# dojo-sim/ContactImplicitMPC.jl

Hardware: AMD Instinct MI355X
Metric: MPC steps/s (quadruped, H=40, fp64) (higher is better)
Workload: dtype f64

## Files before the change

contactimplicitmpc/jl_amd/csrc/cimpc_host.cpp:

```cpp
#include <hip/hip_runtime.h>

#include <algorithm>
#include <chrono>
#include <cmath>
#include <cstdio>
#include <cstdlib>
#include <cstring>
#include <string>
#include <vector>

#include "cimpc_internal.h"
#include "lin_table.h"
#include "lin_table_build.h"
#include "model_table.h"
#include "newton_state.h"
#include "gains.h"
#include "handle_state.h"
#include "plant_linearize.h"
#include "schedule_plan.h"

using namespace cimpc;

namespace {

// ... 26 lines not shown
    int kkt_tw_spins = 0;
    int banded_form = 0;

    static int env_int(const char* name, int dflt) { const char* v = getenv(name); return v ? atoi(v) : dflt; }
    void read_environment() {
        sched.async_mode = env_int("CIMPC_ASYNC", sched.async_mode);
        sched.async_tail = env_int("CIMPC_ASYNC_TAIL", sched.async_tail);
        sched.spec_first = env_int("CIMPC_SPEC_FIRST", sched.spec_first);
        sched.iter_cap = std::max(1, env_int("CIMPC_ITER_CAP", sched.iter_cap));
        async_debug = getenv("CIMPC_ASYNC_DEBUG") != nullptr;
        if (const char* v = getenv("CIMPC_ASYNC_WATCHDOG_S")) watchdog_s = atof(v);
        debug_rounds = getenv("CIMPC_DEBUG_ROUNDS") != nullptr;
        sched.tail_div = env_int("CIMPC_TAIL_DIV", sched.tail_div);
        sched.async_full_max = env_int("CIMPC_ASYNC_FULL_MAX", sched.async_full_max);
        sched.drain_pct = env_int("CIMPC_DRAIN_PCT", sched.drain_pct);
        sched.drain_min = std::max(1, env_int("CIMPC_DRAIN_MIN", sched.drain_min));
        kkt.kkt_pipe = env_int("CIMPC_KKT_PIPE", kkt.kkt_pipe);
        kkt.kkt_twisted = env_int("CIMPC_KKT_TWISTED", kkt.kkt_twisted);
        kkt_tw_nb = env_int("CIMPC_KKT_TW_NB", kkt_tw_nb);
        kkt.lazy_dz = env_int("CIMPC_LAZY_DZ", 1) != 0;
        kkt.kkt_duo = env_int("CIMPC_KKT_DUO", kkt.kkt_duo);
        kkt.kkt_duo_hint = env_int("CIMPC_KKT_DUO_HINT", kkt.kkt_duo_hint);
        kkt.async_kkt_tw = env_int("CIMPC_ASYNC_KKT_TW", kkt.async_kkt_tw);
        generic_static = env_int("CIMPC_GENERIC_STATIC", generic_static ? 1 : 0) != 0;
        sched.sweep_wgs = env_int("CIMPC_SWEEP_WGS", sched.sweep_wgs);
        sched.waves32 = env_int("CIMPC_WAVES32", sched.waves32);
        banded_form = env_int("CIMPC_BANDED_FORM", banded_form);
    }
};

struct cimpc_ctx {
    cimpc_dims dm{};
    Knobs kn{};
    cimpc_ip_opts ip{};
    cimpc_newton_opts nt{};
    int device = 0;
    hipStream_t stream = nullptr;
    bool own_stream = false;
    std::string err;
    KernelInfo ki{};
    int nz = 0, nth = 0, nths = 0, nd = 0, nr = 0, nx = 0, ny = 0, N = 0;
// ... 1056 lines not shown
    if (from_reset) h->prof_kkt_systems += h->last_stats.newton_iters;
    return CIMPC_OK;
}

int launch_round(cimpc_ctx* h, SolveRun& run, long long r, bool blind) {
    const RoundStreams& sb = run.sb; const RoundCounts& last = run.last;
    const int par = (int)(r & 1);
    h->S.kkt_tw_epoch += 1;
    const bool tw_off = note_tw_fallbacks(h) != run.tw_fail0;
    NewtonDev Sk = launch_view(h, par);
    Sk.A.n_done = run.hybrid ? h->a_ctrl + async_ctl(h->Q.K).n_done : nullptr;
    Sk.round_stamp = (int)(r + 1);
    const bool kkt = (r > 0) && (blind || last.kkt > 0);
    const int n_kkt = blind ? h->dm.B : last.kkt;
    const int* n_kkt_dev = blind ? round_counter(Sk.counters_next, RC_KKT) : nullptr;
    if (kkt) {
        const bool ov = h->kp.kkt_overlap;
        const KktSite site{.kind = ov ? KktSite::Overlapped : KktSite::Round, .n_kkt = n_kkt, .blind = blind,
                           .sweep_problems = (long long)last.new_slots * h->dm.H, .tw_off = tw_off, .B = h->dm.B};
        hipStream_t kst = ov ? sb.st_kkt : sb.st;
        if (!ov) Sk.kkt_same_round = 1;
        prof_begin(h, PC_KKT, kst);
        int rk = run_kkt_stage(h, Sk, kkt_newton_args(Sk), site, Sk.kkt_list + (size_t)(par ^ 1) * h->dm.B,
                               ov ? last.kkt : n_kkt, ov ? nullptr : n_kkt_dev, kst);
        prof_end(h, kst);
        if (rk != CIMPC_OK) return fail(h, rk, "kkt launch failed");
        if (ov && hipEventRecord(sb.ev_join, sb.st_kkt) != hipSuccess) return fail(h, CIMPC_ERR_HIP, "join record failed");
    }
    const RoundPlan rp = plan_round(h->kn.sched, h->sched, h->ip.max_iter, kkt, blind, last.sweep, last.slots);
    const long long hint = blind ? -1 : (long long)last.slots * h->dm.H + last.parked;
    if (h->kn.debug_rounds && !blind) print_queued_problems(h, run, r, par, hint);
    int rr = run_sweep(h, par, round_counter(Sk.counters, RC_PARKED), nullptr, sb.st, rp.cap, round_counter(Sk.counters, RC_DRAINED), true, hint);
    if (rr != CIMPC_OK) return rr;
    prof_begin(h, PC_RESID, sb.st);
    if (rp.split_join) {
        rr = launch_resid_decide(Sk, sb.st, rp.n_slots, 1);
        if (rr != CIMPC_OK) return fail(h, rr, "residual launch failed");
    }
    if (kkt && h->kp.kkt_overlap && hipStreamWaitEvent(sb.st, sb.ev_join, 0) != hipSuccess) return fail(h, CIMPC_ERR_HIP, "join failed");
    rr = launch_resid_decide(Sk, sb.st, rp.n_slots, rp.split_join ? 2 : 0);
    prof_end(h, sb.st);
    if (rr != CIMPC_OK) return fail(h, rr, "residual launch failed");
    return CIMPC_OK;
}

}

int cimpc_newton_solve_dev(cimpc_handle h, const double* q0_dev, const double* q1_dev, int warm_start) {
    int rc = check_ready(h, true);
    if (rc != CIMPC_OK) return rc;
    if (!q0_dev || !q1_dev) return fail(h, CIMPC_ERR_INVALID, "null argument");
    HIP_TRY(h, hipSetDevice(h->device));
    if (int sy = sync_dz_stores(h, DZ_NEWTON); sy != CIMPC_OK) return sy;
    h->st.solve_started();
// ... 25 lines not shown
    while (true) {
        if (completed >= round_limit) {
            (void)hipStreamSynchronize(sb.st); (void)hipStreamSynchronize(sb.st_kkt);
            return fail(h, CIMPC_ERR_STATE, "newton_solve: round limit reached with unfinished rollouts");
        }
        while (launched <= completed + (ahead ? 1 : 0)) {
            rc = launch_round(h, run, launched, launched > completed);
            if (rc != CIMPC_OK) return rc;
            ++launched;
        }
        {
            volatile int* hm = ring_slot((volatile int*)h->h_ring, completed);
            const int want = (int)(completed + 1);
            long long spins = 0;
            while (hm[RING_STAMP] != want) {
                if ((++spins & 0xFFFFF) == 0 && hipStreamQuery(sb.st) != hipErrorNotReady && hm[RING_STAMP] != want)
                    return fail(h, CIMPC_ERR_HIP, "round finished without publishing its counters");
            }
        }
        const RoundCounts& last = run.last = read_round_counts(h->h_ring, completed);
        if (h->kn.debug_rounds) fprintf(stderr, "[cimpc round %lld] t %.3f ms: next sweep %d rollouts (%d evaluation slots), next kkt %d, parked %d, finished %d\n", completed,
                                        1e3 * elapsed_s(run), last.sweep, last.slots, last.kkt, last.parked, last.finished);
        h->prof_kkt_systems += last.kkt;
        ++completed;
        if ((last.sweep == 0 && last.kkt == 0) || over_budget(h, run)) break;
        if (run.hybrid && hand_over(h->sched, B - last.finished)) {
            HIP_TRY(h, hipStreamSynchronize(sb.st));
            HIP_TRY(h, hipStreamSynchronize(sb.st_kkt));
            return run_async(h, run, false, completed);
        }
    }
// ... 377 lines not shown
```

contactimplicitmpc/jl_amd/csrc/newton_impl.h:

```cpp
#pragma once
#include "lane_group.h"
#include "newton_state.h"

namespace cimpc {

struct BlockSync { static __device__ __forceinline__ void sync() { __syncthreads(); } };
struct WaveSync {
    static __device__ __forceinline__ void sync() {
        __builtin_amdgcn_fence(__ATOMIC_SEQ_CST, "workgroup");
        __builtin_amdgcn_wave_barrier();
    }
};

__device__ __forceinline__ void theta_update(const NewtonDev& S, const TrajDev& T, int b, int i,
                                             int tid, int nthreads) {
    const cimpc_dims& m = S.dm;
    double* th = T.th + ((size_t)b * m.H + i) * S.nth;
    const double* q = T.q + ((size_t)b * (m.H + 2) + i) * m.nq;
    const double* u = T.u + ((size_t)b * m.H + i) * m.nu;
    const double* w = T.w + ((size_t)b * m.H + i) * m.nw;
    for (int k = tid; k < 2 * m.nq; k += nthreads) th[k] = q[k];
    for (int k = tid; k < m.nu; k += nthreads) th[2 * m.nq + k] = u[k];
    for (int k = tid; k < m.nw; k += nthreads) th[2 * m.nq + m.nu + k] = w[k];
}
// ... 13 lines not shown

__device__ __forceinline__ void enqueue_eval(const NewtonDev& S, size_t sb, int b, int par, int tid, int nt, int list_pos = -1) {
    const int H = S.dm.H, K = S.WQ.K;
    for (int k = tid; k < H; k += nt) {
        const int t = S.WQ.window[(size_t)b * (H + 2) + k];
        const int pos = atomicAdd(qcount(S.WQ, par, t), 1);
        S.WQ.items[((size_t)par * K + t) * S.WQ.cap + pos] = (int)(sb * H + k);
    }
    if (tid == 0) {
        S.WQ.done_count[sb] = 0;
        S.need_sweep[sb] = 1;
        list_slot(S, sb, par, list_pos);
    }
}

__device__ __forceinline__ void enqueue_evals(const NewtonDev& S, size_t sb, int n, int b, int par, int tid, int nt, int mark = 1) {
    const int H = S.dm.H, K = S.WQ.K;
    for (int k = tid; k < H; k += nt) {
        const int t = S.WQ.window[(size_t)b * (H + 2) + k];
        const int pos = atomicAdd(qcount(S.WQ, par, t), n);
        int* it = S.WQ.items + ((size_t)par * K + t) * S.WQ.cap + pos;
        for (int c = 0; c < n; ++c) it[c] = (int)((sb + c) * H + k);
    }
    if (tid == 0) {
        int pos = 0;
        if (S.slot_list != nullptr) pos = atomicAdd(round_counter(S.counters, RC_SLOTS), n);
        atomicAdd(round_counter(S.counters, RC_NEW_SLOTS), n);
        if (pos + n > S.dm.B * CS) __builtin_trap();
        for (int c = 0; c < n; ++c) {
            S.WQ.done_count[sb + c] = 0;
            S.need_sweep[sb + c] = mark;
// ... 157 lines not shown
}

template <class Sync>
__device__ __forceinline__ void start_line_search(const NewtonDev& S, int b, int mode, int lane, int nt) {
    const size_t sb0 = (size_t)b * CS;
    int n = 1;
    {
        const int prev = S.ls_iter[b];
        if (S.newton_l[b] == 0) n = S.spec_first;
        else if (prev >= S.spec_all) n = 7;
        else if (prev >= S.spec_mid) n = 3;
        n = (n >= 7) ? 7 : (n >= 3) ? 3 : 1;
    }
    Sync::sync();
    apply_steps<Sync>(S, sb0, 0, n, b, lane, nt);
    if (lane == 0) { S.alpha[b] = 1.0; S.ls_iter[b] = 0; S.stage[b] = (n == 7) ? STAGE_LS7 : (n == 3) ? STAGE_LS3 : STAGE_LS0; }
    if (mode == 2) {
        enqueue_eval_async<Sync>(S, sb0, 0, n, b, lane, nt);
    } else {
        const int par = (S.kkt_same_round == 1) ? S.WQ.par : (S.WQ.par ^ 1);
        enqueue_evals(S, sb0, n, b, par, lane, nt, S.kkt_same_round == 0 ? 2 : 1);
        if (lane == 0) {
            for (int c = n; c < CS; ++c) S.need_sweep[sb0 + c] = 0;
            if (S.kkt_same_round == 0) atomicAdd(round_counter(S.counters, RC_SWEEP), 1);
        }
    }
}


__device__ __forceinline__ const double* dz_eff(const NewtonDev& S, int b, int it, int i) {
    const int H = S.dm.H;
    const size_t sb0 = (size_t)b * CS, blk = (size_t)S.nths * S.nd;
    int s = it;
    while (s >= 0 && S.ip_status[(sb0 + s) * H + i] == 0) --s;
    return s >= 0 ? S.dz + ((sb0 + s) * H + i) * blk : S.dz_good + ((size_t)b * H + i) * blk;
}

template <int NQ, int NU, bool CF>
__device__ double slot_residual(const NewtonDev& S, size_t sb, int b, const int* eff, int tid, int nt, double* absr = nullptr) {
// ... 183 lines not shown
        for (int k = tid; k < K; k += nt) { *qcount(S.WQ, par, k) = 0; *qhead(S.WQ, k) = 0; }
        if (tid < ROUND_COUNTERS) *round_counter(S.counters_next, tid) = 0;
    }
    RPROF_BEGIN(1)
    int pre_dc = H, pre_ns = 0;
    double pre_rc = 0.0;
    if constexpr (SPLIT == 2) {
        if (tid < CS) { pre_dc = S.WQ.done_count[sb0 + tid]; pre_ns = S.need_sweep[sb0 + tid]; pre_rc = S.r_cand[sb0 + tid]; }
    }
    const int stage = S.stage[b];
    if (stage == STAGE_DONE || stage == STAGE_KKT) return;
    const int ncand = (stage == STAGE_LS1) ? 2 : (stage == STAGE_LS2) ? 4 : (stage == STAGE_LS7) ? 7 : (stage == STAGE_LS3) ? 3 : 1;
    const int it0 = (stage == STAGE_LS1) ? 1 : (stage == STAGE_LS2) ? 3 : 0;
    if constexpr (SPLIT == 2) {
        const bool mine = tid >= it0 && tid < it0 + ncand;
        if (!__syncthreads_or(tid == it0 && pre_ns != 0)) return;
        if (__syncthreads_or(tid == it0 && pre_ns == 2)) {
            if (mine) S.need_sweep[sb0 + tid] = 1;
            return;
        }
        if (__syncthreads_or(mine && pre_dc < H)) {
            if (tid == 0) atomicAdd(round_counter(S.counters, RC_SWEEP), 1);
            if (mine) list_slot(S, sb0 + tid, S.WQ.par ^ 1);
            return;
        }
        if (mine) rc[tid - it0] = pre_rc;
    } else {
        if (S.need_sweep[sb0 + it0] == 0) return;
        if constexpr (!ASYNC) {
            if (S.need_sweep[sb0 + it0] == 2) {
                __syncthreads();
                if (tid < ncand) S.need_sweep[sb0 + it0 + tid] = 1;
                return;
            }
        }
        if constexpr (!ASYNC) {
            int pend = 0;
            if (tid < ncand) pend = (S.WQ.done_count[sb0 + it0 + tid] < H);
            if (__syncthreads_or(pend)) {
                if (tid == 0) atomicAdd(round_counter(S.counters, RC_SWEEP), 1);
                return;
            }
        }
    }
    int& s_act = sh[0]; int& s_slot = sh[1]; int& s_iter = sh[2];
    constexpr int EFF_H = 128;
    __shared__ int eff[(SPLIT ? 1 : CS) * EFF_H];
    const bool use_eff = H <= EFF_H;
    auto resolve_eff = [&](int c, int* row) {
        for (int i = tid; i < H && use_eff; i += nt) {
            int s_ = it0 + c;
            while (s_ >= 0 && S.ip_status[(sb0 + s_) * H + i] == 0) --s_;
            row[i] = s_;
        }
    };
// ... 179 lines not shown
        sh[3] = done;
    }
    if constexpr (ASYNC) {
        xfence(S.A.flags);
        __syncthreads();
        if (tid == 0) {
            if (sh[3]) {
                if (atomicAdd(S.A.n_done, 1) == S.A.B - 1) wake_all(S.A);
            } else {
                push_kkt_job(S.A, b);
            }
        }
    }
}

#define CIMPC_KKT_PRIO 2
#define CIMPC_RESID_THREADS 256
#define CIMPC_SLOT_THREADS 256
template <int NQ, int NU, bool CF>
__global__ __launch_bounds__(CIMPC_SLOT_THREADS) void resid_slot_kernel(NewtonDev S, const int* list) {
    constexpr int CT = 256, EFF_H = 128;
    extern __shared__ __attribute__((aligned(16))) double red[];
    __shared__ int eff[EFF_H];
    const int tid = threadIdx.x, nt = blockDim.x, H = S.dm.H;
    RPROF_BEGIN(0)
    int my, b;
    if (list != nullptr) {
        const int e = list[blockIdx.x];
        b = e / CS; my = e - b * CS;
    } else {
// ... 1 lines not shown
    }
    const size_t sb0 = (size_t)b * CS, sb = sb0 + my;
    const bool use_eff = H <= EFF_H;
    const int ns_my = S.need_sweep[sb];
    const int stage = S.stage[b];
    const int dc = tid < CS ? S.WQ.done_count[sb0 + tid] : H;
    const int nsl = tid < CS ? S.need_sweep[sb0 + tid] : 0;
    int eff_i = -1;
    if (use_eff && tid < H) {
#pragma unroll
        for (int s_ = 0; s_ < CS; ++s_) {
            const int ok = (s_ <= my) ? S.ip_status[(sb0 + s_) * H + tid] : 0;
            if (ok != 0) eff_i = s_;
        }
    }
    if (ns_my != 1 || stage == STAGE_DONE || stage == STAGE_KKT) return;
    const int ncand = (stage == STAGE_LS1) ? 2 : (stage == STAGE_LS2) ? 4 : (stage == STAGE_LS7) ? 7 : (stage == STAGE_LS3) ? 3 : 1;
    const int it0 = (stage == STAGE_LS1) ? 1 : (stage == STAGE_LS2) ? 3 : 0;
    if (my < it0 || my >= it0 + ncand) return;
    const bool mine = tid >= it0 && tid < it0 + ncand;
    if (__syncthreads_or((tid == it0 && nsl != 1) || (mine && dc < H))) return;
    if (use_eff && tid < H) eff[tid] = eff_i;
    __syncthreads();
    RPROF(1)
    if (S.N <= SLOT_ABS_MAX) {
        double* absr = red + CT;
        slot_residual<NQ, NU, CF>(S, sb, b, use_eff ? eff : nullptr, tid, nt, absr);
        __syncthreads();
        RPROF(2)
        if (tid < CT) {
            double part = 0.0;
            for (int e = tid; e < S.N; e += CT) part += absr[e];
            red[tid] = part;
        }
    } else {
        const double part = tid < CT ? slot_residual<NQ, NU, CF>(S, sb, b, use_eff ? eff : nullptr, tid, CT) : 0.0;
// ... 1 lines not shown
    }
    __syncthreads();
    for (int st = CT / 2; st > 0; st >>= 1) {
        if (tid < st) red[tid] += red[tid + st];
        __syncthreads();
    }
    if (tid == 0) S.r_cand[sb] = red[0];
    RPROF(3)
}
template <int NQ, int NU, bool CF, bool SINGLE = false>
__global__ __launch_bounds__(CIMPC_RESID_THREADS) void resid_decide_kernel(NewtonDev S) {
    extern __shared__ __attribute__((aligned(16))) double red[];
    __shared__ double rc[CS];
    __shared__ int sh[4];
    resid_decide_body<NQ, NU, CF, false, SINGLE ? 0 : 2>(S, (int)blockIdx.x + S.b0, red, rc, sh);
    __syncthreads();
    if (threadIdx.x == 0) {
        __threadfence();
        const int ticket = atomicAdd(round_counter(S.counters, RC_TICKET), 1);
        if (ticket == (int)gridDim.x - 1) {
            const int n_sweep = atomicAdd(round_counter(S.counters, RC_SWEEP), 0), n_kkt = atomicAdd(round_counter(S.counters, RC_KKT), 0);
            volatile int* hm = S.host_flag;
            hm[RING_N_SWEEP] = n_sweep;
            hm[RING_N_KKT] = n_kkt;
            hm[RING_PARKED] = atomicAdd(round_counter(S.counters, RC_PARKED), 0);
            hm[RING_SLOTS] = atomicAdd(round_counter(S.counters, RC_SLOTS), 0);
            hm[RING_NEW_SLOTS] = atomicAdd(round_counter(S.counters, RC_NEW_SLOTS), 0);
            hm[RING_FINISHED] = S.A.n_done != nullptr ? atomicAdd(S.A.n_done, 0) : 0;
            __threadfence_system();
            hm[RING_STAMP] = S.round_stamp;
            __threadfence_system();
        }
    }
}

__device__ __forceinline__ const double* kkt_dz(const NewtonDev& S, const KktArgs& K, int b, int H, int nths, int nd) {
    if (K.dz_override) return K.dz_override + (size_t)b * H * nths * nd;
    return K.stage ? S.dz_good + (size_t)b * H * nths * nd : S.dz + (size_t)b * CS * H * nths * nd;
}

__device__ __forceinline__ void lds_sync() { __syncthreads(); }

constexpr int KKT_TILES = 21;

template <int NQ, int NU>
__global__ __launch_bounds__(64) void kkt_kernel_scalar(NewtonDev S, KktArgs K) {
    constexpr int LD = ((NQ > NU ? NQ : NU) + 3) & ~3;
    const cimpc_dims& m = S.dm;
// ... 1138 lines not shown


#define CIMPC_KKT_PACK 2
#define CIMPC_KKT_PACK_WAVES_PER_SIMD 2
constexpr int KKT_PACK = CIMPC_KKT_PACK;
template <int NQ, int NU>
constexpr int kkt_pack() {
    constexpr int fit = (160 * 1024 / 8) / kkt_lds_doubles<NQ, NU, 1>();
    return fit < 1 ? 1 : (fit < KKT_PACK ? fit : KKT_PACK);
}
template <int NQ, int NU>
__global__ __launch_bounds__((64 * kkt_pack<NQ, NU>()), (kkt_tld<NQ, NU>() <= 16 ? CIMPC_KKT_PACK_WAVES_PER_SIMD : 1)) void kkt_kernel_packed(NewtonDev S, KktArgs K, const int* list, int n, const int* n_dev) {
    extern __shared__ __attribute__((aligned(16))) double sm[];
    if (n_dev != nullptr) n = *n_dev;
    const int wave = (int)threadIdx.x >> 6, slot = (int)blockIdx.x * kkt_pack<NQ, NU>() + wave;
    if (slot >= n) return;
    __builtin_amdgcn_s_setprio(CIMPC_KKT_PRIO);
    kkt_body<NQ, NU, WaveSync>(S, K, list[slot], sm + (size_t)wave * kkt_lds_doubles<NQ, NU, 1>(), (int)threadIdx.x & 63);
}

template <int NQ, int NU>
__global__ __launch_bounds__(192, (kkt_tld<NQ, NU>() <= 16 ? 2 : 1)) void kkt_kernel_pipe(NewtonDev S, KktArgs K, const int* list, int n, const int* n_dev) {
    extern __shared__ __attribute__((aligned(16))) double sm[];
    if (n_dev != nullptr) n = *n_dev;
    if ((int)blockIdx.x >= n) return;
    kkt_body<NQ, NU, WaveSync, 3>(S, K, list[blockIdx.x], sm, (int)threadIdx.x & 63, (int)threadIdx.x >> 6);
}

struct KktTwArgs { NewtonDev S; KktArgs K; const int* list; int n; const int* n_dev; };
template <class T, size_t OFFSET>
__device__ __forceinline__ T kkt_kernarg(unsigned long long v) {
    T out;
#if defined(__HIP_DEVICE_COMPILE__)
    const unsigned lo = __builtin_amdgcn_readfirstlane((unsigned)v);
    const unsigned hi = __builtin_amdgcn_readfirstlane((unsigned)(v >> 32));
    const unsigned long long u = (((unsigned long long)hi << 32) | lo) + OFFSET;
    __builtin_memcpy(&out, (const __attribute__((address_space(4))) T*)u, sizeof(T));
#else
    (void)v;
#endif
    return out;
}
using lds_double_ptr = __attribute__((address_space(3))) double*;
template <int NQ, int NU, int TW>
static __device__ __attribute__((noinline, noreturn)) void kkt_tw_chain(unsigned long long ka, int b, lds_double_ptr sm3) {
    const NewtonDev S = kkt_kernarg<NewtonDev, offsetof(KktTwArgs, S)>(ka);
    const KktArgs K = kkt_kernarg<KktArgs, offsetof(KktTwArgs, K)>(ka);
    kkt_body<NQ, NU, WaveSync, 3, false, TW>(S, K, b, (double*)sm3, (int)threadIdx.x & 63, (int)threadIdx.x >> 6);
    __builtin_amdgcn_endpgm();
}
template <int NQ, int NU>
__global__ __launch_bounds__(192, (kkt_tld<NQ, NU>() <= 16 ? 2 : 1)) void kkt_kernel_twisted(KktTwArgs A) {
#ifdef CIMPC_KKT_TWPROF
    if (threadIdx.x == 0 && blockIdx.x < 2) ((long long*)A.S.stats)[48 + blockIdx.x] = (long long)wall_clock64();
#endif
    int n = A.n;
    if (A.n_dev != nullptr) n = *A.n_dev;
    const int k = (int)blockIdx.x >> 1;
    if (k >= n) return;
    const int b = A.list != nullptr ? A.list[k] : k + A.S.b0;
    if (A.list == nullptr) {
        if (A.K.stage != nullptr && A.K.stage[b] != STAGE_KKT) return;
        if (A.K.only_flag != nullptr && A.K.only_flag[b] == 0) return;
    }
    extern __shared__ __attribute__((aligned(16))) double sm[];
    const unsigned long long ka = (unsigned long long)__builtin_amdgcn_kernarg_segment_ptr();
    if (((int)blockIdx.x & 1) == 0) kkt_tw_chain<NQ, NU, 2>(ka, b, (lds_double_ptr)sm);
    else kkt_tw_chain<NQ, NU, 1>(ka, b, (lds_double_ptr)sm);
}

template <int NQ, int NU, int TW>
static __device__ __attribute__((noinline, noreturn)) void kkt_duo_chain(unsigned long long ka, int b, lds_double_ptr sm3) {
    const NewtonDev S = kkt_kernarg<NewtonDev, offsetof(KktTwArgs, S)>(ka);
    const KktArgs K = kkt_kernarg<KktArgs, offsetof(KktTwArgs, K)>(ka);
    kkt_body<NQ, NU, WaveSync, 1, false, TW>(S, K, b, (double*)sm3, (int)threadIdx.x & 63, 0);
    __builtin_amdgcn_endpgm();
}
template <int NQ, int NU>
__global__ __launch_bounds__(128, CIMPC_KKT_PACK_WAVES_PER_SIMD) void kkt_kernel_duo(KktTwArgs A) {
    int n = A.n;
    if (A.n_dev != nullptr) n = *A.n_dev;
    const int k = (int)blockIdx.x;
    if (k >= n) return;
    const int b = A.list != nullptr ? A.list[k] : k + A.S.b0;
    if (A.list == nullptr) {
        if (A.K.stage != nullptr && A.K.stage[b] != STAGE_KKT) return;
        if (A.K.only_flag != nullptr && A.K.only_flag[b] == 0) return;
    }
    extern __shared__ __attribute__((aligned(16))) double sm[];
    __builtin_amdgcn_s_setprio(CIMPC_KKT_PRIO);
    const unsigned long long ka = (unsigned long long)__builtin_amdgcn_kernarg_segment_ptr();
    if (((int)threadIdx.x >> 6) == 0) kkt_duo_chain<NQ, NU, 2>(ka, b, (lds_double_ptr)sm);
    else kkt_duo_chain<NQ, NU, 1>(ka, b, (lds_double_ptr)(sm + kkt_duo_slice_doubles(2)));
}

template <int NQ, int NU, bool F32 = false>
__global__ __launch_bounds__(64, (kkt_tld<NQ, NU>() <= 16 ? 2 : 1)) void kkt_kernel(NewtonDev S, KktArgs K) {
    extern __shared__ __attribute__((aligned(16))) double sm[];
// ... 8 lines not shown
```

contactimplicitmpc/jl_amd/csrc/newton_kernels.hip:

```cpp
#include <cstdlib>
#ifdef CIMPC_KKT_PROF
#define CIMPC_KKT_WPROF
#endif
#include "newton_impl.h"
#include "model_table.h"

namespace cimpc {

__global__ __launch_bounds__(256) void reset_kernel(NewtonDev S, const double* q0,
                                                    const double* q1, int warm) {
    const cimpc_dims& m = S.dm;
    const int b = blockIdx.x + S.b0, tid = threadIdx.x, nt = blockDim.x;
    const int H = m.H;
    const size_t oq = (size_t)b * (H + 2) * m.nq;
    const size_t sb0 = (size_t)b * CS;
    if (!warm) {
        for (int k = tid; k < H * S.nd; k += nt) {
            S.nu[(size_t)b * H * S.nd + k] = 0.0;
        }
        copy_n(S.traj.q + oq, S.ref.q + oq, (H + 2) * m.nq, tid, nt);
        copy_n(S.traj.u + (size_t)b * H * m.nu, S.ref.u + (size_t)b * H * m.nu, H * m.nu, tid, nt);
        copy_n(S.traj.w + (size_t)b * H * m.nw, S.ref.w + (size_t)b * H * m.nw, H * m.nw, tid, nt);
        copy_n(S.traj.g + (size_t)b * H * m.nc, S.ref.g + (size_t)b * H * m.nc, H * m.nc, tid, nt);
        copy_n(S.traj.b + (size_t)b * H * m.nb, S.ref.b + (size_t)b * H * m.nb, H * m.nb, tid, nt);
// ... 45 lines not shown
        if (f32) return launch_lds(optin32, kkt_kernel<NQ, NU, true>, dim3(S.nb_launch), dim3(64), lds, s, S, K);
        return launch_lds(optin, kkt_kernel<NQ, NU>, dim3(S.nb_launch), dim3(64), lds, s, S, K);
    }
    if (f != KktForm::Scalar || f32) return CIMPC_ERR_INVALID;
    constexpr int LD = ((NQ > NU ? NQ : NU) + 3) & ~3;
    static LdsOptIn optin;
    return launch_lds(optin, kkt_kernel_scalar<NQ, NU>, dim3(S.nb_launch), dim3(64), (size_t)(KKT_TILES * LD * LD + 10 * LD) * sizeof(double), s, S, K);
}

template <int NQ, int NU>
static int launch_kkt_list_t(const NewtonDev& S, const KktArgs& K, KktForm f, const int* list, int n, const int* n_dev, hipStream_t s) {
    if constexpr (NQ <= 24 && NU <= 24) {
        if (S.dm.H > kkt_max_h<NQ, NU>()) return CIMPC_ERR_INVALID;
        if constexpr (kkt_tld<NQ, NU>() == 16) if (f == KktForm::Duo) {
            static LdsOptIn optin;
            return launch_lds(optin, kkt_kernel_duo<NQ, NU>, dim3(n), dim3(128), (size_t)(kkt_duo_slice_doubles(1) + kkt_duo_slice_doubles(2)) * sizeof(double),
                              s, KktTwArgs{S, K, list, n, n_dev});
        }
        if (f == KktForm::Twisted) {
            static LdsOptIn optin;
            return launch_lds(optin, kkt_kernel_twisted<NQ, NU>, dim3(2 * n), dim3(192), (size_t)kkt_tw_lds_doubles<NQ, NU>() * sizeof(double), s,
                              KktTwArgs{S, K, list, n, n_dev});
        }
        if (f == KktForm::Pipelined && list != nullptr) {
            static LdsOptIn optin;
            return launch_lds(optin, kkt_kernel_pipe<NQ, NU>, dim3(n), dim3(192), (size_t)kkt_lds_doubles<NQ, NU, 3>() * sizeof(double), s, S, K, list, n, n_dev);
        }
        if (f == KktForm::Packed && list != nullptr) {
            constexpr int PACK = kkt_pack<NQ, NU>();
            static LdsOptIn optin;
            return launch_lds(optin, kkt_kernel_packed<NQ, NU>, dim3((n + PACK - 1) / PACK), dim3(64 * PACK), (size_t)PACK * kkt_lds_doubles<NQ, NU, 1>() * sizeof(double),
                              s, S, K, list, n, n_dev);
        }
    }
    return CIMPC_ERR_INVALID;
}
static int launch_kkt_condensed(const NewtonDev& S, const KktArgs& K, KktForm f, bool f32, const int* list, int n, const int* n_dev, hipStream_t s) {
    if (S.dm.mode != CIMPC_MODE_CONFIGURATION) return CIMPC_ERR_INVALID;
    const bool rollout = f == KktForm::PerRollout || f == KktForm::Scalar;
    if (n_dev != nullptr) n = S.dm.B;
    if (n <= 0) return CIMPC_OK;
    const int nq = S.dm.nq, nu = S.dm.nu;
#define X(name, q, u, w, c, b, a) if (nq == q && nu == u) return rollout ? launch_kkt_t<q, u>(S, K, f, f32, s) : f32 ? CIMPC_ERR_INVALID : launch_kkt_list_t<q, u>(S, K, f, list, n, n_dev, s);
    CIMPC_MODEL_TABLE(X)
#undef X
    return CIMPC_ERR_INVALID;
}

__device__ __forceinline__ double kkt_apply_row(const NewtonDev& S, const double* dzb, const double* x, double rho, int e) {
    const int H = S.dm.H, nq = S.dm.nq, nu = S.dm.nu, nr = nq + nu, nd = nq, blk = (2 * nq + nu) * nd;
// ... 492 lines not shown
```

contactimplicitmpc/jl_amd/csrc/newton_state.h:

```cpp
#pragma once
#include "cimpc_internal.h"
#include "kkt_plan.h"

namespace cimpc {
constexpr int NLOG = 16;

enum Stage : int { STAGE_DONE = 0, STAGE_INIT = 1, STAGE_LS0 = 2, STAGE_KKT = 3, STAGE_LS1 = 4, STAGE_LS2 = 5, STAGE_LS7 = 6, STAGE_LS3 = 7 };
constexpr int CS = 7;

struct TrajDev {
    double* q;
    double* u;
    double* w;
    double* g;
    double* b;
    double* th;
};

struct NewtonDev {
    cimpc_dims dm;
    int b0;
    int nb_launch;
    int kkt_same_round;
    int nd, nr, nth, nths, N;
// ... 17 lines not shown
    double* delta;
    double* r_norm;
    double* r_cand;
    double* alpha;
    double* beta;
    int* ls_iter;
    int* newton_l;
    int* stage;
    int* kkt_list;
    int* need_sweep;
    int* slot_list;
    int* counters;
    int* counters_next;
    int* host_flag;
    int round_stamp;
    int band_reduce;
    int band_form;
    long long* stats;
    int* ro_sweeps;
    int* ro_ip_iters;
    int* ro_ip_fail;
    const double* Q;
    const double* R;
    const double* Qinv;
    const double* Rinv;
    const double* Cg;
    const double* Cb;
    const double* V;
    const double* q_target;
    const double* v_target;
// ... 31 lines not shown
struct KktArgs {
    const double* r;
    double* delta;
    const double* beta;
    double beta_scalar;
    const int* stage;
    int finish;
    const double* dz_override;
    const int* only_flag;
};
inline KktArgs kkt_newton_args(const NewtonDev& S) { return KktArgs{S.res, S.delta, S.beta, 0.0, S.stage, 1, nullptr, nullptr}; }
inline KktArgs kkt_raw_args(const double* r, double beta, double* delta) { return KktArgs{r, delta, nullptr, beta, nullptr, 0, nullptr, nullptr}; }
struct KktWorkspace { double* dense; double* cf; double* mix; int* mix_nfb; };
int launch_kkt_stage(const NewtonDev& S, const KktArgs& K, KktBackend be, KktForm f, const int* list, int n, const int* n_dev,
                     const KktWorkspace& W, hipStream_t s);
bool kkt_condensed_available(const NewtonDev& nd);
bool kkt_mfma_available(const NewtonDev& nd);
bool kkt_packed_available(const NewtonDev& nd);
bool kkt_twisted_available(const NewtonDev& nd);
bool kkt_duo_available(const NewtonDev& nd);
bool kkt_mixed_available(const NewtonDev& nd);
bool kkt_banded_available(const NewtonDev& S);
bool kkt_banded_twisted_available(const NewtonDev& S);
bool kkt_cf_reduce_available(const NewtonDev& S);
size_t kkt_mixed_workspace_doubles(const NewtonDev& nd);
size_t kkt_dense_workspace_doubles(const NewtonDev& S, bool banded);
size_t cf_reduce_doubles(const NewtonDev& S);
NewtonDev cf_shadow(const NewtonDev& S);
int launch_queue_recycle(const IpQueues& Q, int par, hipStream_t s);
int launch_solve_finish(const NewtonDev& nd, double* out, hipStream_t s);
// ... 4 lines not shown
```

contactimplicitmpc/jl_amd/csrc/round_protocol.h:

```cpp
#pragma once
#include <stddef.h>

#if defined(__HIPCC__)
#define ROUND_HD __host__ __device__ __forceinline__
#else
#define ROUND_HD inline
#endif

namespace cimpc {

constexpr int QPAD = 32;
constexpr int CPAD = 32;

enum RoundCounter : int {
    RC_SWEEP = 0,
    RC_KKT = 1,
    RC_PARKED = 2,
    RC_DRAINED = 3,
    RC_SLOTS = 4,
    RC_NEW_SLOTS = 5,
    RC_TICKET = 7,
};
constexpr int ROUND_COUNTERS = 8;
constexpr int ROUND_COUNTER_INTS = ROUND_COUNTERS * CPAD;
ROUND_HD constexpr int* round_counter(int* block, int k) { return block + k * CPAD; }
ROUND_HD constexpr int* round_counter_block(int* blocks, int parity) { return blocks + ROUND_COUNTER_INTS * parity; }

enum RingWord : int {
    RING_N_SWEEP = 0,
    RING_N_KKT = 1,
    RING_STAMP = 2,
    RING_ABORT = 3,
    RING_PARKED = 4,
    RING_FINISHED = 5,
    RING_SLOTS = 6,
    RING_NEW_SLOTS = 7,
};
constexpr int RING_SLOT_INTS = 8, RING_SLOTS_COUNT = 2, RING_ALLOC_INTS = 32;
constexpr RingWord RING_PUBLISHED[] = {RING_N_SWEEP, RING_N_KKT, RING_PARKED, RING_SLOTS, RING_NEW_SLOTS, RING_FINISHED, RING_STAMP};
template <class T> ROUND_HD constexpr T* ring_slot(T* ring, long long round) { return ring + RING_SLOT_INTS * (round & 1); }
template <class T> ROUND_HD constexpr T* ring_abort_word(T* ring) { return ring + RING_ABORT; }
// ... 45 lines not shown
```

contactimplicitmpc/jl_amd/csrc/schedule_plan.h:

```cpp
#pragma once
#include <algorithm>
#include <cstddef>
#include "kkt_plan.h"

namespace cimpc {

struct SchedulePolicy {
    int async_mode = 2;
    int async_tail = -1;
    int async_full_max = 32;
    int spec_first = -1;
    int iter_cap = 28;
    int tail_div = 8;
    int drain_pct = 95;
    int drain_min = 4;
    int sweep_wgs = 0;
    int waves32 = 0;
};
struct ScheduleFacts {
    int B = 1, H = 1, H_ref = 1, G = 16;
    bool async_available = false;
};
struct SchedulePlan {
    ScheduleFacts f;
    bool async_on = false, single_launch = false, hybrid = false;
    int async_tail = 96;
    int waves = 4, wpk = 1;
    long long adapt32 = 0;
    int async_grid = 0, async_service = 0;
    int tail_grid = 0, tail_service = 0;
    int spec_all = 3, spec_first = 3, spec_mid = 8, spec_tail = 3;
    bool kkt_overlap = false;
};
constexpr int async_idle_sleep = 2, async_idle_spins = 48, async_wake_fan = 1;

inline SchedulePlan plan_schedule(const SchedulePolicy& p, const ScheduleFacts& f) {
    SchedulePlan s;
    const int B = (s.f = f).B;
    s.async_on = p.async_mode != 0 && f.async_available;
    s.single_launch = s.async_on && (p.async_mode == 1 || (p.async_mode == 2 && B >= 4 && B <= p.async_full_max));
    s.hybrid = s.async_on && p.async_mode == 2 && !s.single_launch && B > p.async_full_max;
    s.async_tail = p.async_tail >= 0 ? p.async_tail : f.G == 32 ? 16 : B < 256 ? std::max(32, B / 4) : std::min(96, std::max(64, B / 6));
    s.spec_all = B <= 128 ? 3 : 8;
    s.spec_first = p.spec_first >= 0 ? p.spec_first : (B <= 1024 ? 3 : 1);
    s.spec_mid = B > 128 ? 1 : 8;
    s.kkt_overlap = B >= 64;
    if (f.G == 32) {
        if (p.waves32 > 0 && p.waves32 < 1000) s.waves = p.waves32;
        else if ((size_t)B * f.H >= 6000) s.waves = 8;
        s.adapt32 = p.waves32 >= 1000 ? p.waves32 : (p.waves32 == 4 || p.waves32 == 8) ? 0 : 7000;
    }
    if (s.single_launch) s.waves = 4;
    const size_t groups_per_wg = (64 / f.G) * s.waves;
    const size_t nprob = (size_t)B * f.H;
    size_t w = (nprob + 2 * groups_per_wg - 1) / (2 * groups_per_wg);
    w = std::max<size_t>(w, std::min<size_t>(f.H_ref, nprob));
    const size_t resident = (size_t)256 * std::max(1, (f.G == 16 ? (s.waves > 4 ? 2 * s.waves : 8) : 4) / s.waves);
    s.wpk = p.sweep_wgs > 0 ? p.sweep_wgs : (int)std::max<size_t>(1, std::min<size_t>(w, resident));
    const int a_wgs = p.sweep_wgs > 0 ? s.wpk : std::max(s.wpk, 240);
    s.async_service = std::max(1, a_wgs / 8);
    s.async_grid = std::max((int)std::min<size_t>(resident, (size_t)a_wgs + s.async_service), s.async_service + 1);
// ... 1 lines not shown
    s.tail_grid = std::min(tail, s.async_grid);
    s.tail_service = tail < s.async_grid ? std::max(1, tail / 8) : s.async_service;
    return s;
}

enum class SolvePath { Rounds, Persistent, Hybrid };
inline SolvePath choose_solve_path(const SchedulePlan& s, KktBackend be) {
    return be != KktBackend::Condensed ? SolvePath::Rounds : s.single_launch ? SolvePath::Persistent : s.hybrid ? SolvePath::Hybrid : SolvePath::Rounds;
}
inline int max_rounds(const SchedulePolicy& p, int newton_max_iter, int ip_max_iter) {
    const int min_progress = p.drain_pct > 0 ? std::min(p.iter_cap, p.drain_min) : p.iter_cap;
    return (newton_max_iter * 8 + 2) * ((ip_max_iter + min_progress - 1) / min_progress + 1);
}

inline bool round_ahead(const SchedulePlan& s, KktBackend be, bool warm_start, bool budget) { return s.f.B < 4 && be != KktBackend::CondensedMixed && warm_start && !budget; }
struct RoundPlan { int cap, n_slots; bool split_join; };
inline RoundPlan plan_round(const SchedulePolicy& p, const SchedulePlan& s, int ip_max_iter, bool kkt, bool blind, int last_sweep, int last_slots) {
    const bool sparse = p.tail_div > 0 && (s.f.B < p.tail_div || (!blind && (long long)last_sweep * p.tail_div <= s.f.B));
    const int cap = sparse ? ip_max_iter : p.iter_cap;
    const int n_slots = s.kkt_overlap ? last_slots : (s.f.B < 4 ? -2 : -1);
    return {cap, n_slots, kkt && s.kkt_overlap && n_slots >= 0};
}

inline bool hand_over(const SchedulePlan& s, int active) { return active > 0 && active <= s.async_tail; }
struct SweepLaunch { int waves, wpk; bool direct; int drain_thresh; };
inline SweepLaunch plan_sweep(const SchedulePolicy& p, const SchedulePlan& s, long long hint, int iter_cap, int ip_max_iter, bool drain) {
    SweepLaunch l{s.waves, s.wpk, false, 0};
    if (s.adapt32 > 0 && hint > 0 && s.kkt_overlap && p.sweep_wgs <= 0) {
        l.waves = hint >= s.adapt32 ? 8 : 4;
        const size_t groups_per_wg = 2 * (size_t)l.waves;
        size_t w = ((size_t)hint + 2 * groups_per_wg - 1) / (2 * groups_per_wg);
        w = std::max<size_t>(w, std::min<size_t>((size_t)s.f.H_ref, (size_t)std::max<long long>(hint, 1)));
        l.wpk = (int)std::max<size_t>(1, std::min<size_t>(w, 256));
    }
    if (s.f.B < 4 && p.sweep_wgs <= 0) { l.direct = true; l.wpk = s.f.H_ref; }
    if (drain && p.drain_pct > 0 && iter_cap < ip_max_iter) l.drain_thresh = std::max(1, (int)((long long)l.wpk * p.drain_pct / 100));
// ... 5 lines not shown
```

Measured before the change: 74980.

## Replace KKT/residual stream join with shared completion ticket for round publish

Removes the event-based join between the overlapped KKT stream and the residual stream. KKT kernels and residual-decide blocks now share one atomic ticket counter, and whichever workgroup finishes last publishes the round counters to the host. Need-sweep marks are now tagged with round parity so residual blocks can tell which round a mark belongs to. This takes a cross-stream dependency off the critical path, at the cost of more complex completion logic and a possible race if the ticket counts are wrong.

Result: faster. 76630, median of 6 (+2.2%).

```diff
diff --git a/contactimplicitmpc/jl_amd/csrc/cimpc_host.cpp b/contactimplicitmpc/jl_amd/csrc/cimpc_host.cpp
--- a/contactimplicitmpc/jl_amd/csrc/cimpc_host.cpp
+++ b/contactimplicitmpc/jl_amd/csrc/cimpc_host.cpp
@@ -64,7 +64,6 @@
         sched.tail_div = env_int("CIMPC_TAIL_DIV", sched.tail_div);
         sched.async_full_max = env_int("CIMPC_ASYNC_FULL_MAX", sched.async_full_max);
         sched.drain_pct = env_int("CIMPC_DRAIN_PCT", sched.drain_pct);
-        sched.drain_min = std::max(1, env_int("CIMPC_DRAIN_MIN", sched.drain_min));
         kkt.kkt_pipe = env_int("CIMPC_KKT_PIPE", kkt.kkt_pipe);
         kkt.kkt_twisted = env_int("CIMPC_KKT_TWISTED", kkt.kkt_twisted);
         kkt_tw_nb = env_int("CIMPC_KKT_TW_NB", kkt_tw_nb);
@@ -75,6 +74,7 @@
         generic_static = env_int("CIMPC_GENERIC_STATIC", generic_static ? 1 : 0) != 0;
         sched.sweep_wgs = env_int("CIMPC_SWEEP_WGS", sched.sweep_wgs);
         sched.waves32 = env_int("CIMPC_WAVES32", sched.waves32);
+        sched.round_join = env_int("CIMPC_ROUND_JOIN", sched.round_join);
         banded_form = env_int("CIMPC_BANDED_FORM", banded_form);
     }
 };
@@ -1161,30 +1161,38 @@
     const bool kkt = (r > 0) && (blind || last.kkt > 0);
     const int n_kkt = blind ? h->dm.B : last.kkt;
     const int* n_kkt_dev = blind ? round_counter(Sk.counters_next, RC_KKT) : nullptr;
+    const bool ov = h->kp.kkt_overlap;
+    const int n_kkt_list = ov ? last.kkt : n_kkt;
+    KktForm form = KktForm::PerRollout;
     if (kkt) {
-        const bool ov = h->kp.kkt_overlap;
         const KktSite site{.kind = ov ? KktSite::Overlapped : KktSite::Round, .n_kkt = n_kkt, .blind = blind,
                            .sweep_problems = (long long)last.new_slots * h->dm.H, .tw_off = tw_off, .B = h->dm.B};
+        form = plan_kkt_stage(h, site);
+    }
+    const int kkt_wgs = kkt && ov && !blind ? kkt_ticket_workgroups(Sk, h->kb, form, n_kkt_list) : 0;
+    const RoundPlan rp = plan_round(h->kn.sched, h->sched, h->ip.max_iter, kkt, blind, last.sweep, last.slots, kkt_wgs);
+    Sk.kkt_ticket = kkt && ov && !rp.join ? 1 : 0;
+    Sk.round_tickets = round_tickets(Sk.nb_launch, Sk.kkt_ticket ? kkt_wgs : 0);
+    if (kkt) {
         hipStream_t kst = ov ? sb.st_kkt : sb.st;
         if (!ov) Sk.kkt_same_round = 1;
         prof_begin(h, PC_KKT, kst);
-        int rk = run_kkt_stage(h, Sk, kkt_newton_args(Sk), site, Sk.kkt_list + (size_t)(par ^ 1) * h->dm.B,
-                               ov ? last.kkt : n_kkt, ov ? nullptr : n_kkt_dev, kst);
+        int rk = launch_kkt_stage(Sk, kkt_newton_args(Sk), h->kb, form, Sk.kkt_list + (size_t)(par ^ 1) * h->dm.B, n_kkt_list, ov ? nullptr : n_kkt_dev,
+                                  KktWorkspace{h->d_dense_ws, h->d_cf_ws, h->d_mix_ws, h->d_mix_nfb}, kst);
         prof_end(h, kst);
         if (rk != CIMPC_OK) return fail(h, rk, "kkt launch failed");
-        if (ov && hipEventRecord(sb.ev_join, sb.st_kkt) != hipSuccess) return fail(h, CIMPC_ERR_HIP, "join record failed");
-    }
-    const RoundPlan rp = plan_round(h->kn.sched, h->sched, h->ip.max_iter, kkt, blind, last.sweep, last.slots);
+    }
     const long long hint = blind ? -1 : (long long)last.slots * h->dm.H + last.parked;
     if (h->kn.debug_rounds && !blind) print_queued_problems(h, run, r, par, hint);
     int rr = run_sweep(h, par, round_counter(Sk.counters, RC_PARKED), nullptr, sb.st, rp.cap, round_counter(Sk.counters, RC_DRAINED), true, hint);
     if (rr != CIMPC_OK) return rr;
+    if (rp.join && hipEventRecord(sb.ev_join, sb.st_kkt) != hipSuccess) return fail(h, CIMPC_ERR_HIP, "join record failed");
     prof_begin(h, PC_RESID, sb.st);
     if (rp.split_join) {
         rr = launch_resid_decide(Sk, sb.st, rp.n_slots, 1);
         if (rr != CIMPC_OK) return fail(h, rr, "residual launch failed");
     }
-    if (kkt && h->kp.kkt_overlap && hipStreamWaitEvent(sb.st, sb.ev_join, 0) != hipSuccess) return fail(h, CIMPC_ERR_HIP, "join failed");
+    if (rp.join && hipStreamWaitEvent(sb.st, sb.ev_join, 0) != hipSuccess) return fail(h, CIMPC_ERR_HIP, "join failed");
     rr = launch_resid_decide(Sk, sb.st, rp.n_slots, rp.split_join ? 2 : 0);
     prof_end(h, sb.st);
     if (rr != CIMPC_OK) return fail(h, rr, "residual launch failed");
@@ -1240,7 +1248,7 @@
             const int want = (int)(completed + 1);
             long long spins = 0;
             while (hm[RING_STAMP] != want) {
-                if ((++spins & 0xFFFFF) == 0 && hipStreamQuery(sb.st) != hipErrorNotReady && hm[RING_STAMP] != want)
+                if ((++spins & 0xFFFFF) == 0 && hipStreamQuery(sb.st) != hipErrorNotReady && hipStreamQuery(sb.st_kkt) != hipErrorNotReady && hm[RING_STAMP] != want)
                     return fail(h, CIMPC_ERR_HIP, "round finished without publishing its counters");
             }
         }
diff --git a/contactimplicitmpc/jl_amd/csrc/newton_impl.h b/contactimplicitmpc/jl_amd/csrc/newton_impl.h
--- a/contactimplicitmpc/jl_amd/csrc/newton_impl.h
+++ b/contactimplicitmpc/jl_amd/csrc/newton_impl.h
@@ -51,7 +51,7 @@
     }
 }
 
-__device__ __forceinline__ void enqueue_evals(const NewtonDev& S, size_t sb, int n, int b, int par, int tid, int nt, int mark = 1) {
+__device__ __forceinline__ void enqueue_evals(const NewtonDev& S, size_t sb, int n, int b, int par, int tid, int nt, int mark = NEED_EVAL) {
     const int H = S.dm.H, K = S.WQ.K;
     for (int k = tid; k < H; k += nt) {
         const int t = S.WQ.window[(size_t)b * (H + 2) + k];
@@ -239,15 +239,21 @@
     }
     Sync::sync();
     apply_steps<Sync>(S, sb0, 0, n, b, lane, nt);
-    if (lane == 0) { S.alpha[b] = 1.0; S.ls_iter[b] = 0; S.stage[b] = (n == 7) ? STAGE_LS7 : (n == 3) ? STAGE_LS3 : STAGE_LS0; }
+    const int nstage = (n == 7) ? STAGE_LS7 : (n == 3) ? STAGE_LS3 : STAGE_LS0;
+    if (lane == 0) { S.alpha[b] = 1.0; S.ls_iter[b] = 0; }
     if (mode == 2) {
+        if (lane == 0) S.stage[b] = nstage;
         enqueue_eval_async<Sync>(S, sb0, 0, n, b, lane, nt);
     } else {
         const int par = (S.kkt_same_round == 1) ? S.WQ.par : (S.WQ.par ^ 1);
-        enqueue_evals(S, sb0, n, b, par, lane, nt, S.kkt_same_round == 0 ? 2 : 1);
+        enqueue_evals(S, sb0, n, b, par, lane, nt, S.kkt_same_round == 0 ? need_mark_overlapped(S.WQ.par) : NEED_EVAL);
         if (lane == 0) {
             for (int c = n; c < CS; ++c) S.need_sweep[sb0 + c] = 0;
-            if (S.kkt_same_round == 0) atomicAdd(round_counter(S.counters, RC_SWEEP), 1);
+            if (S.kkt_same_round == 0) {
+                atomicAdd(round_counter(S.counters, RC_SWEEP), 1);
+                __threadfence();
+            }
+            S.stage[b] = nstage;
         }
     }
 }
@@ -461,31 +467,25 @@
     const int it0 = (stage == STAGE_LS1) ? 1 : (stage == STAGE_LS2) ? 3 : 0;
     if constexpr (SPLIT == 2) {
         const bool mine = tid >= it0 && tid < it0 + ncand;
-        if (!__syncthreads_or(tid == it0 && pre_ns != 0)) return;
-        if (__syncthreads_or(tid == it0 && pre_ns == 2)) {
-            if (mine) S.need_sweep[sb0 + tid] = 1;
-            return;
-        }
+        if (!__syncthreads_or(tid == it0 && need_is_mine(pre_ns, S.WQ.par))) return;
         if (__syncthreads_or(mine && pre_dc < H)) {
             if (tid == 0) atomicAdd(round_counter(S.counters, RC_SWEEP), 1);
-            if (mine) list_slot(S, sb0 + tid, S.WQ.par ^ 1);
+            if (mine) { S.need_sweep[sb0 + tid] = NEED_EVAL; list_slot(S, sb0 + tid, S.WQ.par ^ 1); }
             return;
         }
         if (mine) rc[tid - it0] = pre_rc;
     } else {
-        if (S.need_sweep[sb0 + it0] == 0) return;
+        const int ns0 = S.need_sweep[sb0 + it0];
+        if (ns0 == 0) return;
         if constexpr (!ASYNC) {
-            if (S.need_sweep[sb0 + it0] == 2) {
-                __syncthreads();
-                if (tid < ncand) S.need_sweep[sb0 + it0 + tid] = 1;
-                return;
-            }
+            if (!need_is_mine(ns0, S.WQ.par)) return;
         }
         if constexpr (!ASYNC) {
             int pend = 0;
             if (tid < ncand) pend = (S.WQ.done_count[sb0 + it0 + tid] < H);
             if (__syncthreads_or(pend)) {
                 if (tid == 0) atomicAdd(round_counter(S.counters, RC_SWEEP), 1);
+                if (tid < ncand) S.need_sweep[sb0 + it0 + tid] = NEED_EVAL;
                 return;
             }
         }
@@ -695,6 +695,28 @@
     }
 }
 
+__device__ __forceinline__ void publish_round(const NewtonDev& S) {
+    const int n_sweep = atomicAdd(round_counter(S.counters, RC_SWEEP), 0), n_kkt = atomicAdd(round_counter(S.counters, RC_KKT), 0);
+    volatile int* hm = S.host_flag;
+    hm[RING_N_SWEEP] = n_sweep;
+    hm[RING_N_KKT] = n_kkt;
+    hm[RING_PARKED] = atomicAdd(round_counter(S.counters, RC_PARKED), 0);
+    hm[RING_SLOTS] = atomicAdd(round_counter(S.counters, RC_SLOTS), 0);
+    hm[RING_NEW_SLOTS] = atomicAdd(round_counter(S.counters, RC_NEW_SLOTS), 0);
+    hm[RING_FINISHED] = S.A.n_done != nullptr ? atomicAdd(S.A.n_done, 0) : 0;
+    __threadfence_system();
+    hm[RING_STAMP] = S.round_stamp;
+    __threadfence_system();
+}
+__device__ __forceinline__ void round_ticket(const NewtonDev& S) {
+    __syncthreads();
+    if (threadIdx.x == 0) {
+        __threadfence();
+        const int ticket = atomicAdd(round_counter(S.counters, RC_TICKET), 1);
+        if (last_ticket(ticket, S.round_tickets)) publish_round(S);
+    }
+}
+
 #define CIMPC_KKT_PRIO 2
 #define CIMPC_RESID_THREADS 256
 #define CIMPC_SLOT_THREADS 256
@@ -726,12 +748,13 @@
             if (ok != 0) eff_i = s_;
         }
     }
-    if (ns_my != 1 || stage == STAGE_DONE || stage == STAGE_KKT) return;
+    const int par = S.WQ.par;
+    if (!need_is_mine(ns_my, par) || stage == STAGE_DONE || stage == STAGE_KKT) return;
     const int ncand = (stage == STAGE_LS1) ? 2 : (stage == STAGE_LS2) ? 4 : (stage == STAGE_LS7) ? 7 : (stage == STAGE_LS3) ? 3 : 1;
     const int it0 = (stage == STAGE_LS1) ? 1 : (stage == STAGE_LS2) ? 3 : 0;
     if (my < it0 || my >= it0 + ncand) return;
     const bool mine = tid >= it0 && tid < it0 + ncand;
-    if (__syncthreads_or((tid == it0 && nsl != 1) || (mine && dc < H))) return;
+    if (__syncthreads_or((tid == it0 && !need_is_mine(nsl, par)) || (mine && dc < H))) return;
     if (use_eff && tid < H) eff[tid] = eff_i;
     __syncthreads();
     RPROF(1)
@@ -763,24 +786,7 @@
     __shared__ double rc[CS];
     __shared__ int sh[4];
     resid_decide_body<NQ, NU, CF, false, SINGLE ? 0 : 2>(S, (int)blockIdx.x + S.b0, red, rc, sh);
-    __syncthreads();
-    if (threadIdx.x == 0) {
-        __threadfence();
-        const int ticket = atomicAdd(round_counter(S.counters, RC_TICKET), 1);
-        if (ticket == (int)gridDim.x - 1) {
-            const int n_sweep = atomicAdd(round_counter(S.counters, RC_SWEEP), 0), n_kkt = atomicAdd(round_counter(S.counters, RC_KKT), 0);
-            volatile int* hm = S.host_flag;
-            hm[RING_N_SWEEP] = n_sweep;
-            hm[RING_N_KKT] = n_kkt;
-            hm[RING_PARKED] = atomicAdd(round_counter(S.counters, RC_PARKED), 0);
-            hm[RING_SLOTS] = atomicAdd(round_counter(S.counters, RC_SLOTS), 0);
-            hm[RING_NEW_SLOTS] = atomicAdd(round_counter(S.counters, RC_NEW_SLOTS), 0);
-            hm[RING_FINISHED] = S.A.n_done != nullptr ? atomicAdd(S.A.n_done, 0) : 0;
-            __threadfence_system();
-            hm[RING_STAMP] = S.round_stamp;
-            __threadfence_system();
-        }
-    }
+    round_ticket(S);
 }
 
 __device__ __forceinline__ const double* kkt_dz(const NewtonDev& S, const KktArgs& K, int b, int H, int nths, int nd) {
@@ -1949,17 +1955,19 @@
     extern __shared__ __attribute__((aligned(16))) double sm[];
     if (n_dev != nullptr) n = *n_dev;
     const int wave = (int)threadIdx.x >> 6, slot = (int)blockIdx.x * kkt_pack<NQ, NU>() + wave;
-    if (slot >= n) return;
-    __builtin_amdgcn_s_setprio(CIMPC_KKT_PRIO);
-    kkt_body<NQ, NU, WaveSync>(S, K, list[slot], sm + (size_t)wave * kkt_lds_doubles<NQ, NU, 1>(), (int)threadIdx.x & 63);
+    if (slot < n) {
+        __builtin_amdgcn_s_setprio(CIMPC_KKT_PRIO);
+        kkt_body<NQ, NU, WaveSync>(S, K, list[slot], sm + (size_t)wave * kkt_lds_doubles<NQ, NU, 1>(), (int)threadIdx.x & 63);
+    }
+    if (S.kkt_ticket) round_ticket(S);
 }
 
 template <int NQ, int NU>
 __global__ __launch_bounds__(192, (kkt_tld<NQ, NU>() <= 16 ? 2 : 1)) void kkt_kernel_pipe(NewtonDev S, KktArgs K, const int* list, int n, const int* n_dev) {
     extern __shared__ __attribute__((aligned(16))) double sm[];
     if (n_dev != nullptr) n = *n_dev;
-    if ((int)blockIdx.x >= n) return;
-    kkt_body<NQ, NU, WaveSync, 3>(S, K, list[blockIdx.x], sm, (int)threadIdx.x & 63, (int)threadIdx.x >> 6);
+    if ((int)blockIdx.x < n) kkt_body<NQ, NU, WaveSync, 3>(S, K, list[blockIdx.x], sm, (int)threadIdx.x & 63, (int)threadIdx.x >> 6);
+    if (S.kkt_ticket) round_ticket(S);
 }
 
 struct KktTwArgs { NewtonDev S; KktArgs K; const int* list; int n; const int* n_dev; };
@@ -1982,6 +1990,7 @@
     const NewtonDev S = kkt_kernarg<NewtonDev, offsetof(KktTwArgs, S)>(ka);
     const KktArgs K = kkt_kernarg<KktArgs, offsetof(KktTwArgs, K)>(ka);
     kkt_body<NQ, NU, WaveSync, 3, false, TW>(S, K, b, (double*)sm3, (int)threadIdx.x & 63, (int)threadIdx.x >> 6);
+    if (S.kkt_ticket) round_ticket(S);
     __builtin_amdgcn_endpgm();
 }
 template <int NQ, int NU>
@@ -1992,7 +2001,7 @@
     int n = A.n;
     if (A.n_dev != nullptr) n = *A.n_dev;
     const int k = (int)blockIdx.x >> 1;
-    if (k >= n) return;
+    if (k >= n) { if (A.S.kkt_ticket) round_ticket(A.S); return; }
     const int b = A.list != nullptr ? A.list[k] : k + A.S.b0;
     if (A.list == nullptr) {
         if (A.K.stage != nullptr && A.K.stage[b] != STAGE_KKT) return;
@@ -2009,6 +2018,7 @@
     const NewtonDev S = kkt_kernarg<NewtonDev, offsetof(KktTwArgs, S)>(ka);
     const KktArgs K = kkt_kernarg<KktArgs, offsetof(KktTwArgs, K)>(ka);
     kkt_body<NQ, NU, WaveSync, 1, false, TW>(S, K, b, (double*)sm3, (int)threadIdx.x & 63, 0);
+    if (S.kkt_ticket) round_ticket(S);
     __builtin_amdgcn_endpgm();
 }
 template <int NQ, int NU>
@@ -2016,7 +2026,7 @@
     int n = A.n;
     if (A.n_dev != nullptr) n = *A.n_dev;
     const int k = (int)blockIdx.x;
-    if (k >= n) return;
+    if (k >= n) { if (A.S.kkt_ticket) round_ticket(A.S); return; }
     const int b = A.list != nullptr ? A.list[k] : k + A.S.b0;
     if (A.list == nullptr) {
         if (A.K.stage != nullptr && A.K.stage[b] != STAGE_KKT) return;
diff --git a/contactimplicitmpc/jl_amd/csrc/newton_kernels.hip b/contactimplicitmpc/jl_amd/csrc/newton_kernels.hip
--- a/contactimplicitmpc/jl_amd/csrc/newton_kernels.hip
+++ b/contactimplicitmpc/jl_amd/csrc/newton_kernels.hip
@@ -83,26 +83,44 @@
         if (S.dm.H > kkt_max_h<NQ, NU>()) return CIMPC_ERR_INVALID;
         if constexpr (kkt_tld<NQ, NU>() == 16) if (f == KktForm::Duo) {
             static LdsOptIn optin;
-            return launch_lds(optin, kkt_kernel_duo<NQ, NU>, dim3(n), dim3(128), (size_t)(kkt_duo_slice_doubles(1) + kkt_duo_slice_doubles(2)) * sizeof(double),
+            return launch_lds(optin, kkt_kernel_duo<NQ, NU>, dim3(kkt_grid_duo(n)), dim3(128), (size_t)(kkt_duo_slice_doubles(1) + kkt_duo_slice_doubles(2)) * sizeof(double),
                               s, KktTwArgs{S, K, list, n, n_dev});
         }
         if (f == KktForm::Twisted) {
             static LdsOptIn optin;
-            return launch_lds(optin, kkt_kernel_twisted<NQ, NU>, dim3(2 * n), dim3(192), (size_t)kkt_tw_lds_doubles<NQ, NU>() * sizeof(double), s,
+            return launch_lds(optin, kkt_kernel_twisted<NQ, NU>, dim3(kkt_grid_twisted(n)), dim3(192), (size_t)kkt_tw_lds_doubles<NQ, NU>() * sizeof(double), s,
                               KktTwArgs{S, K, list, n, n_dev});
         }
         if (f == KktForm::Pipelined && list != nullptr) {
             static LdsOptIn optin;
-            return launch_lds(optin, kkt_kernel_pipe<NQ, NU>, dim3(n), dim3(192), (size_t)kkt_lds_doubles<NQ, NU, 3>() * sizeof(double), s, S, K, list, n, n_dev);
+            return launch_lds(optin, kkt_kernel_pipe<NQ, NU>, dim3(kkt_grid_pipelined(n)), dim3(192), (size_t)kkt_lds_doubles<NQ, NU, 3>() * sizeof(double), s, S, K, list, n, n_dev);
         }
         if (f == KktForm::Packed && list != nullptr) {
             constexpr int PACK = kkt_pack<NQ, NU>();
             static LdsOptIn optin;
-            return launch_lds(optin, kkt_kernel_packed<NQ, NU>, dim3((n + PACK - 1) / PACK), dim3(64 * PACK), (size_t)PACK * kkt_lds_doubles<NQ, NU, 1>() * sizeof(double),
+            return launch_lds(optin, kkt_kernel_packed<NQ, NU>, dim3(kkt_grid_packed(n, PACK)), dim3(64 * PACK), (size_t)PACK * kkt_lds_doubles<NQ, NU, 1>() * sizeof(double),
                               s, S, K, list, n, n_dev);
         }
     }
     return CIMPC_ERR_INVALID;
+}
+template <int NQ, int NU>
+static int kkt_ticket_wgs_t(KktForm f, int n) {
+    if constexpr (NQ <= 24 && NU <= 24) {
+        if (f == KktForm::Duo) return kkt_tld<NQ, NU>() == 16 ? kkt_grid_duo(n) : 0;
+        if (f == KktForm::Twisted) return kkt_grid_twisted(n);
+        if (f == KktForm::Pipelined) return kkt_grid_pipelined(n);
+        if (f == KktForm::Packed) return kkt_grid_packed(n, kkt_pack<NQ, NU>());
+    }
+    return 0;
+}
+int kkt_ticket_workgroups(const NewtonDev& S, KktBackend be, KktForm f, int n) {
+    if (be != KktBackend::Condensed || S.dm.mode != CIMPC_MODE_CONFIGURATION || n <= 0) return 0;
+    const int nq = S.dm.nq, nu = S.dm.nu;
+#define X(name, q, u, w, c, b, a) if (nq == q && nu == u) return kkt_ticket_wgs_t<q, u>(f, n);
+    CIMPC_MODEL_TABLE(X)
+#undef X
+    return 0;
 }
 static int launch_kkt_condensed(const NewtonDev& S, const KktArgs& K, KktForm f, bool f32, const int* list, int n, const int* n_dev, hipStream_t s) {
     if (S.dm.mode != CIMPC_MODE_CONFIGURATION) return CIMPC_ERR_INVALID;
diff --git a/contactimplicitmpc/jl_amd/csrc/newton_state.h b/contactimplicitmpc/jl_amd/csrc/newton_state.h
--- a/contactimplicitmpc/jl_amd/csrc/newton_state.h
+++ b/contactimplicitmpc/jl_amd/csrc/newton_state.h
@@ -55,6 +55,8 @@
     int* counters_next;
     int* host_flag;
     int round_stamp;
+    int round_tickets;
+    int kkt_ticket;
     int band_reduce;
     int band_form;
     long long* stats;
@@ -116,6 +118,7 @@
 struct KktWorkspace { double* dense; double* cf; double* mix; int* mix_nfb; };
 int launch_kkt_stage(const NewtonDev& S, const KktArgs& K, KktBackend be, KktForm f, const int* list, int n, const int* n_dev,
                      const KktWorkspace& W, hipStream_t s);
+int kkt_ticket_workgroups(const NewtonDev& S, KktBackend be, KktForm f, int n);
 bool kkt_condensed_available(const NewtonDev& nd);
 bool kkt_mfma_available(const NewtonDev& nd);
 bool kkt_packed_available(const NewtonDev& nd);
diff --git a/contactimplicitmpc/jl_amd/csrc/round_protocol.h b/contactimplicitmpc/jl_amd/csrc/round_protocol.h
--- a/contactimplicitmpc/jl_amd/csrc/round_protocol.h
+++ b/contactimplicitmpc/jl_amd/csrc/round_protocol.h
@@ -25,6 +25,18 @@
 constexpr int ROUND_COUNTER_INTS = ROUND_COUNTERS * CPAD;
 ROUND_HD constexpr int* round_counter(int* block, int k) { return block + k * CPAD; }
 ROUND_HD constexpr int* round_counter_block(int* blocks, int parity) { return blocks + ROUND_COUNTER_INTS * parity; }
+
+ROUND_HD constexpr int kkt_grid_packed(int n, int pack) { return n <= 0 ? 0 : (n + pack - 1) / pack; }
+ROUND_HD constexpr int kkt_grid_pipelined(int n) { return n <= 0 ? 0 : n; }
+ROUND_HD constexpr int kkt_grid_duo(int n) { return n <= 0 ? 0 : n; }
+ROUND_HD constexpr int kkt_grid_twisted(int n) { return n <= 0 ? 0 : 2 * n; }
+ROUND_HD constexpr int round_tickets(int decide_wgs, int kkt_wgs) { return decide_wgs + kkt_wgs; }
+ROUND_HD constexpr bool last_ticket(int ticket, int tickets) { return ticket == tickets - 1; }
+
+constexpr int NEED_EVAL = 1, NEED_NEXT_ROUND = 2;
+ROUND_HD constexpr int need_mark_overlapped(int par) { return NEED_NEXT_ROUND + (par & 1); }
+ROUND_HD constexpr bool need_is_next_round(int v, int par) { return v == need_mark_overlapped(par); }
+ROUND_HD constexpr bool need_is_mine(int v, int par) { return v == NEED_EVAL || v == need_mark_overlapped(par ^ 1); }
 
 enum RingWord : int {
     RING_N_SWEEP = 0,
diff --git a/contactimplicitmpc/jl_amd/csrc/schedule_plan.h b/contactimplicitmpc/jl_amd/csrc/schedule_plan.h
--- a/contactimplicitmpc/jl_amd/csrc/schedule_plan.h
+++ b/contactimplicitmpc/jl_amd/csrc/schedule_plan.h
@@ -16,6 +16,7 @@
     int drain_min = 4;
     int sweep_wgs = 0;
     int waves32 = 0;
+    int round_join = 0;
 };
 struct ScheduleFacts {
     int B = 1, H = 1, H_ref = 1, G = 16;
@@ -31,6 +32,7 @@
     int tail_grid = 0, tail_service = 0;
     int spec_all = 3, spec_first = 3, spec_mid = 8, spec_tail = 3;
     bool kkt_overlap = false;
+    bool round_join = false;
 };
 constexpr int async_idle_sleep = 2, async_idle_spins = 48, async_wake_fan = 1;
 
@@ -45,6 +47,7 @@
     s.spec_first = p.spec_first >= 0 ? p.spec_first : (B <= 1024 ? 3 : 1);
     s.spec_mid = B > 128 ? 1 : 8;
     s.kkt_overlap = B >= 64;
+    s.round_join = p.round_join != 0;
     if (f.G == 32) {
         if (p.waves32 > 0 && p.waves32 < 1000) s.waves = p.waves32;
         else if ((size_t)B * f.H >= 6000) s.waves = 8;
@@ -76,12 +79,15 @@
 }
 
 inline bool round_ahead(const SchedulePlan& s, KktBackend be, bool warm_start, bool budget) { return s.f.B < 4 && be != KktBackend::CondensedMixed && warm_start && !budget; }
-struct RoundPlan { int cap, n_slots; bool split_join; };
-inline RoundPlan plan_round(const SchedulePolicy& p, const SchedulePlan& s, int ip_max_iter, bool kkt, bool blind, int last_sweep, int last_slots) {
+struct RoundPlan { int cap, n_slots; bool split_join, join; };
+inline RoundPlan plan_round(const SchedulePolicy& p, const SchedulePlan& s, int ip_max_iter, bool kkt, bool blind, int last_sweep, int last_slots,
+                            int kkt_ticket_wgs = 0) {
     const bool sparse = p.tail_div > 0 && (s.f.B < p.tail_div || (!blind && (long long)last_sweep * p.tail_div <= s.f.B));
     const int cap = sparse ? ip_max_iter : p.iter_cap;
     const int n_slots = s.kkt_overlap ? last_slots : (s.f.B < 4 ? -2 : -1);
-    return {cap, n_slots, kkt && s.kkt_overlap && n_slots >= 0};
+    const bool overlapped = kkt && s.kkt_overlap;
+    const bool join = overlapped && (s.round_join || blind || n_slots < 0 || kkt_ticket_wgs <= 0);
+    return {cap, n_slots, overlapped && n_slots >= 0, join};
 }
 
 inline bool hand_over(const SchedulePlan& s, int active) { return active > 0 && active <= s.async_tail; }
```
